# schmidtjonathan/Climate2Weather

Measured on AMD Instinct MI355X. Metric: UNet denoise steps/sec (train fwd+bwd+allreduce+AdamW+EMA windows/s), higher is better.
Workload: dtype bf16; 1 GPU; configs/sda_unet.yml default net, 5 vars x window 13 = 65 ch, 128x128, bf16 training step, 128 windows/GPU/step; global_batch=128, parallelism=dp1, params=72132929

## Files before the change

climate2weather_amd/csrc/conv_igemm.hip:

```cpp
#include <cstdlib>

#include "conv_epilogue.h"
#include "knobs.h"
#include "launch.h"

namespace {

constexpr int BN = 128;
constexpr int WBYTES = BN * 128;
constexpr int NSLOT = 3;
template <int NW> struct GCfg {
    static constexpr int BM = 64 * NW;
    static constexpr int NTHREADS = 128 * NW;
    static constexpr int PBYTES = BM * 128;
    static constexpr int ROWS_PER_ROUND = NTHREADS / 8;
    static constexpr int WROUNDS = BN / ROWS_PER_ROUND;
    static constexpr int ROUND_BYTES = NTHREADS * 16;
};

template <typename T> struct Mma;
template <> struct Mma<bf16_t> {
    __device__ static __forceinline__ void run(const u32x4_t& a, const u32x4_t& b, f32x4_t& c) { c = mfma16<bf16_t>(a, b, c); }
};
template <> struct Mma<f16_t> {
    __device__ static __forceinline__ void run(const u32x4_t& a, const u32x4_t& b, f32x4_t& c) { c = mfma16<f16_t>(a, b, c); }
};
template <> struct Mma<float> {
    __device__ static __forceinline__ void run(const u32x4_t& a, const u32x4_t& b, f32x4_t& c) {
#pragma unroll
        for (int s = 0; s < 4; ++s)
            c = __builtin_amdgcn_mfma_f32_16x16x4f32(__uint_as_float(a[s]), __uint_as_float(b[s]), c, 0, 0, 0);
    }
};

template <typename T, int MODE, int NW>
__global__ __launch_bounds__(GCfg<NW>::NTHREADS, 2) void conv_igemm_kernel(const C2wConvArgs p) {
    constexpr int BM = GCfg<NW>::BM, NTHREADS = GCfg<NW>::NTHREADS, PBYTES = GCfg<NW>::PBYTES;
    constexpr int RPR = GCfg<NW>::ROWS_PER_ROUND, WROUNDS = GCfg<NW>::WROUNDS, RB = GCfg<NW>::ROUND_BYTES;
    constexpr int ESZ = sizeof(T);
    constexpr int NT = (MODE == C2W_CONV_1X1) ? 1 : 9;
    constexpr int CK = 128 / ESZ;
    extern __shared__ __attribute__((aligned(16))) char smem[];
    char* const Pbuf = smem;
    char* const Wbuf = smem + NSLOT * PBYTES;

    const int tid = threadIdx.x;
    const int lane = tid & 63;
    const int wid = __builtin_amdgcn_readfirstlane(tid >> 6);
    const int li = lane & 15, lg = lane >> 4;
    const int wm = wid & 1, wn = wid >> 1;

    const int nN = (p.Cout + BN - 1) / BN;
    const int nblk = gridDim.x;
    int L;
    {
        const int bid = blockIdx.x, xcd = bid & 7, q = nblk >> 3, r = nblk & 7;
        L = (xcd < r ? xcd * (q + 1) : r * (q + 1) + (xcd - r) * q) + (bid >> 3);
    }
    const int tn = L % nN, tm = L / nN;
    const int co0 = tn * BN;
    const int HWo = p.Hout * p.Wout;
    const int npix = p.B * HWo;

    bool par = false;
    int pa = 0, pw = 0, psh = 0;
    const int Wh = p.Wout >> 1, HWq = HWo >> 2, nq = npix >> 2;
    if constexpr (MODE == C2W_CONV_TS2) {
        par = ((p.Hout | p.Wout) & 1) == 0 && nq % BM == 0;
        if (par) {
            const int cls = (tm * BM) / nq;
            pa = cls < 2;
            pw = (cls & 1) == 0;
            psh = pa + pw;
        }
    }
    const int b0 = (MODE == C2W_CONV_TS2 && par) ? ((tm * BM) % nq) / HWq : (tm * BM) / HWo;
    const size_t img_bytes = (size_t)p.Hin * p.Win * p.Cin * ESZ;
    size_t xrem = (size_t)(p.B - b0) * img_bytes;
    if (xrem > 0x7fffffffu) xrem = 0x7fffffffu;
    const __amdgpu_buffer_rsrc_t rx = make_rsrc((const char*)p.x + (size_t)b0 * img_bytes, (uint32_t)xrem);
    const __amdgpu_buffer_rsrc_t rw = make_rsrc(p.w, (uint32_t)((size_t)p.wrows * NT * p.Cin * ESZ));

    auto row_pixel = [&](int Q, int& b, int& oh, int& ow) {
        if (MODE == C2W_CONV_TS2 && par) {
            const int qq = Q % nq;
            b = qq / HWq;
            const int rem = qq - b * HWq;
            const int yh = rem / Wh;
            oh = 2 * yh + pa;
            ow = 2 * (rem - yh * Wh) + pw;
        } else {
            b = Q / HWo;
            const int rem = Q - b * HWo;
            oh = rem / p.Wout;
            ow = rem - oh * p.Wout;
        }
    };

    int pb[4], pyx[4];
    uint32_t plc[4];
#pragma unroll
    for (int i = 0; i < 4; ++i) {
        const int q = (tid >> 3) + RPR * i;
        const int Q = tm * BM + q;
        int b, oh, ow;
        row_pixel(Q, b, oh, ow);
        pb[i] = (Q < npix) ? (b - b0) * p.Hin : -1;
        pyx[i] = (oh << 16) | ow;
        plc[i] = (uint32_t)(((tid & 7) ^ (q & 7)) << 4);
    }
    uint32_t wvo[WROUNDS];
#pragma unroll
    for (int i = 0; i < WROUNDS; ++i) {
        const int row = (tid >> 3) + RPR * i;
        wvo[i] = (uint32_t)(co0 + row) * (uint32_t)(NT * p.Cin * ESZ) + (uint32_t)(((tid & 7) ^ (row & 7)) << 4);
    }

    const int nchunk = p.Cin / CK;
    const int NS = (MODE == C2W_CONV_TS2 && par) ? (nchunk << psh) : nchunk * NT;

    auto issue = [&](int s, int buf) {
        int chunk, kh, kw;
        if (MODE == C2W_CONV_TS2 && par) {
            chunk = s >> psh;
            const int ti = s - (chunk << psh);
            kh = pa ? 2 * (ti >> pw) : 1;
            kw = pw ? 2 * (ti & 1) : 1;
        } else {
            chunk = s / NT;
            const int tap0 = s - chunk * NT;
            kh = tap0 / 3;
            kw = tap0 - kh * 3;
        }
        const int tap = kh * 3 + kw;
        char* const pdst = Pbuf + buf * PBYTES + wid * 1024;
#pragma unroll
        for (int i = 0; i < 4; ++i) {
            int ih, iw;
            const bool ok = src_pixel<MODE>(p, pyx[i] >> 16, pyx[i] & 0xffff, kh, kw, ih, iw) && pb[i] >= 0;
            const uint32_t voff = ok ? (uint32_t)(((pb[i] + ih) * p.Win + iw) * p.Cin) * ESZ + plc[i] : C2W_OOB;
            glds16(rx, pdst + i * RB, voff, (uint32_t)chunk * 128u);
        }
        char* const wdst = Wbuf + buf * WBYTES + wid * 1024;
        const uint32_t wso = (uint32_t)(tap * p.Cin + chunk * CK) * ESZ;
#pragma unroll
        for (int i = 0; i < WROUNDS; ++i) glds16(rw, wdst + i * RB, wvo[i], wso);
    };

    uint32_t offA[4], offB[4];
#pragma unroll
    for (int m = 0; m < 4; ++m) {
        const int row = wm * 64 + m * 16 + li;
        offA[m] = (uint32_t)(row * 128 + ((lg ^ (row & 7)) << 4));
    }
#pragma unroll
    for (int n = 0; n < 4; ++n) {
        const int row = wn * 64 + n * 16 + li;
        offB[n] = (uint32_t)(row * 128 + ((lg ^ (row & 7)) << 4));
    }

    f32x4_t acc[4][4];
#pragma unroll
    for (int m = 0; m < 4; ++m)
#pragma unroll
        for (int n = 0; n < 4; ++n) acc[m][n] = (f32x4_t){0.f, 0.f, 0.f, 0.f};

    float bv[4][4];
    epi_load_bias(p, co0 + wm * 64 + lg * 4, bv);
    issue(0, 0);
    if (NS > 1) issue(1, 1);
    int slot = 0;
    for (int s = 0; s < NS; ++s) {
        if (s + 1 < NS) {
            if constexpr (WROUNDS == 2) {
                asm volatile("s_waitcnt vmcnt(6)" ::: "memory");
            } else {
                asm volatile("s_waitcnt vmcnt(8)" ::: "memory");
            }
        } else {
            asm volatile("s_waitcnt vmcnt(0)" ::: "memory");
        }
        asm volatile("s_waitcnt lgkmcnt(0)" ::: "memory");
        __builtin_amdgcn_s_barrier();
        if (s + 2 < NS) issue(s + 2, slot >= 1 ? slot - 1 : NSLOT - 1);
        const char* const Pb = Pbuf + slot * PBYTES;
        const char* const Wb = Wbuf + slot * WBYTES;
#pragma unroll
        for (int ks = 0; ks < 2; ++ks) {
            u32x4_t a[4], b[4];
#pragma unroll
            for (int m = 0; m < 4; ++m) a[m] = *(const u32x4_t*)(Wb + (offA[m] ^ (ks * 64)));
#pragma unroll
            for (int n = 0; n < 4; ++n) b[n] = *(const u32x4_t*)(Pb + (offB[n] ^ (ks * 64)));
#pragma unroll
            for (int m = 0; m < 4; ++m)
#pragma unroll
                for (int n = 0; n < 4; ++n) Mma<T>::run(a[m], b[n], acc[m][n]);
        }
        slot = slot + 1 == NSLOT ? 0 : slot + 1;
    }

    constexpr int OS = BN * ESZ + 16;
    EpiStore<T, BM, NTHREADS> est;
    est.prefetch(p, tid, co0, [&](int row) -> long long {
        const int Q = tm * BM + row;
        if (Q >= npix) return -1;
        if (MODE == C2W_CONV_TS2 && par) {
            int b, oh, ow;
            row_pixel(Q, b, oh, ow);
            return ((long long)b * p.Hout + oh) * p.Wout + ow;
        }
        return (long long)Q;
    });
    __syncthreads();
    char* const O = smem;
    epi_acc_to_lds<T>(O, OS, acc, bv, p.act, wm * 64, wn * 64, li, lg);
    __syncthreads();
    est.finish(p, O, OS, tid);
}

template <typename T, int MODE>
__global__ void conv_naive_kernel(const C2wConvArgs p) {
    constexpr int NT = (MODE == C2W_CONV_1X1) ? 1 : 9;
    const int HWo = p.Hout * p.Wout;
    const long long total = (long long)p.B * HWo * p.Cout;
    for (long long idx = (long long)blockIdx.x * blockDim.x + threadIdx.x; idx < total; idx += (long long)gridDim.x * blockDim.x) {
        const int co = (int)(idx % p.Cout);
        const long long Q = idx / p.Cout;
        const int b = (int)(Q / HWo);
        const int rem = (int)(Q - (long long)b * HWo);
        const int oh = rem / p.Wout, ow = rem - oh * p.Wout;
        float acc = 0.f;
        for (int tap = 0; tap < NT; ++tap) {
            int ih, iw;
            if (!src_pixel<MODE>(p, oh, ow, tap / 3, tap % 3, ih, iw)) continue;
            const T* xp = (const T*)p.x + (((size_t)b * p.Hin + ih) * p.Win + iw) * p.Cin;
            const T* wp = (const T*)p.w + ((size_t)co * NT + tap) * p.Cin;
            if (co >= p.wrows) continue;
            for (int ci = 0; ci < p.Cin; ++ci) acc = fmaf(Elem<T>::ld(wp + ci), Elem<T>::ld(xp + ci), acc);
        }
        if (p.bias && co < p.wrows) acc += p.bias[co];
        if (p.act == C2W_ACT_SILU) acc = silu_f(acc);
        if (p.act == C2W_ACT_RELU) acc = relu_f(acc);
        const size_t off = (size_t)Q * p.ldy + co;
        if (p.mul) {
            float g = Elem<T>::ld((const T*)p.mul + off);
            acc *= (p.mulmode == C2W_MUL_DSILU) ? dsilu_f(g) : g;
        }
        if (p.res) acc += Elem<T>::ld((const T*)p.res + off);
        if (p.act == C2W_ACT_SILU_PAIR && p.y2) {
            Elem<T>::st((T*)p.y + off, acc);
            const float a_ = Elem<T>::ld((const T*)p.y + off);
            Elem<T>::st((T*)p.y + off, silu_f(a_));
            Elem<T>::st((T*)p.y2 + off, dsilu_f(a_));
            continue;
        }
        if (p.act == C2W_ACT_RELU_PAIR && p.y2) {
            Elem<T>::st((T*)p.y + off, acc);
            const float a_ = Elem<T>::ld((const T*)p.y + off);
            Elem<T>::st((T*)p.y + off, relu_f(a_));
            Elem<T>::st((T*)p.y2 + off, a_ > 0.f ? 1.f : 0.f);
            continue;
        }
        Elem<T>::st((T*)p.y + off, acc);
        if (p.y2) Elem<T>::st((T*)p.y2 + off, silu_f(Elem<T>::ld((const T*)p.y + off)));
    }
}

template <typename T, int MODE, int NW>
int launch_tile(const C2wConvArgs& a, long long npix, int nN, hipStream_t st) {
    typedef GCfg<NW> CF;
    constexpr int ESZ = sizeof(T);
    constexpr int lds_loop = NSLOT * (CF::PBYTES + WBYTES), lds_epi = CF::BM * (BN * ESZ + 16);
    constexpr int lds = lds_loop > lds_epi ? lds_loop : lds_epi;
    if (int rc = c2w_lds_optin<conv_igemm_kernel<T, MODE, NW>>(lds)) return rc;
    const int nM = (int)((npix + CF::BM - 1) / CF::BM);
    conv_igemm_kernel<T, MODE, NW><<<nM * nN, CF::NTHREADS, lds, st>>>(a);
    return (int)hipGetLastError();
}

template <typename T, int MODE>
int launch_mode(const C2wConvArgs& a, int naive, hipStream_t st) {
    const long long npix = (long long)a.B * a.Hout * a.Wout;
    if (naive) {
        long long total = npix * a.Cout;
        int grid = (int)((total + 255) / 256 < 65536 ? (total + 255) / 256 : 65536);
        conv_naive_kernel<T, MODE><<<grid, 256, 0, st>>>(a);
        return (int)hipGetLastError();
    }
    const int nN = (a.Cout + BN - 1) / BN;
    const bool small = ((npix + 255) / 256) * nN < c2w_cu_count();
    return small ? launch_tile<T, MODE, 2>(a, npix, nN, st) : launch_tile<T, MODE, 4>(a, npix, nN, st);
}

template <typename T>
int launch_dtype(const C2wConvArgs& a, int naive, hipStream_t st) {
    switch (a.mode) {
        case C2W_CONV_1X1: return launch_mode<T, C2W_CONV_1X1>(a, naive, st);
        case C2W_CONV_S1: return launch_mode<T, C2W_CONV_S1>(a, naive, st);
        case C2W_CONV_S2: return launch_mode<T, C2W_CONV_S2>(a, naive, st);
        case C2W_CONV_UP: return launch_mode<T, C2W_CONV_UP>(a, naive, st);
        case C2W_CONV_TS2: return launch_mode<T, C2W_CONV_TS2>(a, naive, st);
    }
    return C2W_ERR_BAD_ARG;
}

}

namespace {
C2wKnobs read_knobs() {
    C2wKnobs k;
    k.force_gather = getenv("C2W_FORCE_GATHER") != nullptr;
    k.conv_t3 = getenv("C2W_CONV_T3") ? atoi(getenv("C2W_CONV_T3")) : -1;
    k.conv_s2_patch = getenv("C2W_CONV_S2_PATCH") ? atoi(getenv("C2W_CONV_S2_PATCH")) : 0;
    k.ts2_pairs = !(getenv("C2W_TS2_PAIRS") && atoi(getenv("C2W_TS2_PAIRS")) == 0);
    k.wgrad_atomics = getenv("C2W_WGRAD_ATOMICS") != nullptr;
    k.loss_fusion = getenv("C2W_NO_LOSS_FUSION") == nullptr;
    k.half8 = getenv("C2W_NO_HALF8") == nullptr;
    k.half8_db = !(getenv("C2W_HALF8_DB") && atoi(getenv("C2W_HALF8_DB")) == 0);
    k.attn_valu = getenv("C2W_ATTN_VALU") != nullptr;
    return k;
}
C2wKnobs g_knobs = read_knobs();
}
const C2wKnobs& c2w_knobs() { return g_knobs; }
extern "C" void c2w_knobs_reload(void) { g_knobs = read_knobs(); }

extern "C" int c2w_conv_patch_supported(const C2wConvArgs* a, int dtype) {
    (void)dtype;
    return a != nullptr && c2w_conv_patch_eligible(*a) && !c2w_knobs().force_gather ? 1 : 0;
}

extern "C" int c2w_conv_pool2_supported(const C2wConvArgs* a, int dtype) {
    (void)dtype;
    if (a == nullptr || a->mode != C2W_CONV_S1 || a->res != nullptr || a->mul != nullptr || a->y2 != nullptr || a->act != C2W_ACT_NONE ||
        a->ln_x != nullptr || a->lnf_y != nullptr)
        return 0;
    return c2w_conv_patch_eligible(*a) && !c2w_conv_pair_eligible(*a) && !c2w_knobs().force_gather ? 1 : 0;
}

extern "C" int c2w_conv_lnfwd_supported(const C2wConvArgs* a, int dtype) {
    if (a == nullptr || (dtype != C2W_DTYPE_BF16 && dtype != C2W_DTYPE_F16)) return 0;
    if (a->Cout != 128 || a->ldy != 128 || a->mul != nullptr || a->y2 != nullptr || a->act != C2W_ACT_NONE || a->ln_x != nullptr) return 0;
    return c2w_conv_patch_eligible(*a) && !c2w_knobs().force_gather ? 1 : 0;
}

extern "C" int c2w_conv_lnbwd_supported(const C2wConvArgs* a, int dtype) {
    if (a == nullptr || (dtype != C2W_DTYPE_BF16 && dtype != C2W_DTYPE_F16)) return 0;
    if (a->Cout != 128 || a->ldy != 128 || a->mul != nullptr || a->y2 != nullptr || a->act != C2W_ACT_NONE) return 0;
    return c2w_conv_patch_eligible(*a) && !c2w_knobs().force_gather ? 1 : 0;
}

int c2w_conv_splitk_plan_impl(const C2wConvArgs& a, int dtype, unsigned long long* ws_bytes);
extern "C" int c2w_conv_splitk_plan(const C2wConvArgs* a, int dtype, unsigned long long* ws_bytes) {
    if (a == nullptr) return C2W_ERR_BAD_ARG;
    return c2w_conv_splitk_plan_impl(*a, dtype, ws_bytes);
}

extern "C" int c2w_conv_lnfwd_chain_supported(const C2wConvArgs* a, int dtype) {
    if (!c2w_conv_lnfwd_supported(a, dtype)) return 0;
    return a->mode == C2W_CONV_S1 && c2w_conv_patch3_wanted(*a, dtype) ? 1 : 0;
}

extern "C" int c2w_conv_loss_supported(const C2wConvArgs* a, int dtype) {
    if (a == nullptr || (dtype != C2W_DTYPE_BF16 && dtype != C2W_DTYPE_F16)) return 0;
    if (a->mode != C2W_CONV_S1 || a->wrows > 80 || a->Cout > 128 || a->ldy != 128 || a->res != nullptr || a->mul != nullptr || a->y2 != nullptr ||
        a->act != C2W_ACT_NONE || a->ln_x != nullptr || a->lnf_y != nullptr || (a->flags & C2W_CONV_POOL2) != 0)
        return 0;
    if (a->loss_sum != nullptr && (a->loss_eps == nullptr || a->loss_C <= 0 || a->loss_C != a->wrows || (a->loss_lde & 7) != 0 || a->loss_lde < a->loss_C ||
                                   a->loss_lde > 128))
        return 0;
    const C2wKnobs& k = c2w_knobs();
    return !k.force_gather && k.loss_fusion && c2w_conv_patch_eligible(*a) && c2w_conv_patch3_wanted(*a, dtype) ? 1 : 0;
}

extern "C" long long c2w_conv_det_scratch_bytes(const C2wConvArgs* a, int dtype) {
    if (a == nullptr) return C2W_ERR_BAD_ARG;
    if (a->ln_x != nullptr && a->ln_dm != nullptr) {
        if (!c2w_conv_lnbwd_supported(a, dtype)) return C2W_ERR_UNSUPPORTED;
        return (long long)a->B * (a->Hout >> 3) * (a->Wout >> 4) * 128 * (long long)sizeof(float);
    }
    if (a->loss_sum != nullptr) {
        C2wConvArgs g = *a;
        g.loss_sum = nullptr;
        if (!c2w_conv_loss_supported(&g, dtype)) return C2W_ERR_UNSUPPORTED;
        return (long long)a->B * (a->Hout >> 4) * (a->Wout >> 4) * ((a->Cout + 127) / 128) * (long long)sizeof(float);
    }
    return 0;
}

extern "C" int c2w_conv_wpacked_supported(const C2wConvArgs* a, int dtype) {
    if (a == nullptr || (dtype != C2W_DTYPE_BF16 && dtype != C2W_DTYPE_F16)) return 0;
    return !c2w_knobs().force_gather && c2w_conv_patch_eligible(*a) && c2w_conv_patch3_wanted(*a, dtype) ? 1 : 0;
}

extern "C" int c2w_conv_dispatch(const C2wConvArgs* a, int dtype) {
    if (a == nullptr) return C2W_ERR_BAD_ARG;
    const bool gather = c2w_knobs().force_gather;
    if (!gather && c2w_conv_patch_eligible(*a)) return c2w_conv_patch3_wanted(*a, dtype) ? C2W_KERNEL_PATCH_16X16 : C2W_KERNEL_PATCH_8X16;
    if (!gather && c2w_conv_pair_eligible(*a)) return C2W_KERNEL_PATCH_PAIR;
    if (!gather && c2w_conv_ts2_patch_eligible(*a)) return C2W_KERNEL_PATCH_TS2;
    if (!gather && c2w_conv_s2_patch_eligible(*a, dtype)) return C2W_KERNEL_PATCH_S2;
    return C2W_KERNEL_GATHER;
}

extern "C" int c2w_conv_forward(const C2wConvArgs* a, int dtype, int naive, void* stream) {
    if (a == nullptr || a->x == nullptr || a->w == nullptr || a->y == nullptr) return C2W_ERR_BAD_ARG;
    const int esz = dtype == C2W_DTYPE_F32 ? 4 : 2;
    const int ck = 128 / esz;
    if (a->Cin <= 0 || a->Cin % ck != 0) return C2W_ERR_BAD_SHAPE;
    if (a->Cout <= 0 || a->Cout % (16 / esz) != 0 || a->ldy % (16 / esz) != 0) return C2W_ERR_BAD_SHAPE;
    if (a->B <= 0 || a->Hin <= 0 || a->Win <= 0 || a->Hout <= 0 || a->Wout <= 0) return C2W_ERR_BAD_SHAPE;
    if (a->Hout >= 65536 || a->Wout >= 65536) return C2W_ERR_BAD_SHAPE;
    if (a->act < C2W_ACT_NONE || a->act > C2W_ACT_RELU_PAIR) return C2W_ERR_BAD_ARG;
    if ((a->act == C2W_ACT_SILU_PAIR || a->act == C2W_ACT_RELU_PAIR) && a->y2 == nullptr) return C2W_ERR_BAD_ARG;
    hipStream_t st = (hipStream_t)stream;
    if (a->ln_x != nullptr && (naive != 0 || !c2w_conv_lnbwd_supported(a, dtype))) return C2W_ERR_BAD_SHAPE;
    if (a->lnf_y != nullptr && (naive != 0 || !c2w_conv_lnfwd_supported(a, dtype))) return C2W_ERR_BAD_SHAPE;
    if ((a->ln_rstd != nullptr && a->ln_x == nullptr) || (a->lnf_rstd != nullptr && a->lnf_y == nullptr)) return C2W_ERR_BAD_ARG;
    if (a->lnf_mean != nullptr || a->res_rstd != nullptr || a->res_mean != nullptr || a->res_m != nullptr || (a->flags & C2W_CONV_NO_Y) != 0) {
        if (a->lnf_y == nullptr || (a->res_rstd == nullptr) != (a->res_mean == nullptr) || (a->res_m != nullptr && a->res_rstd == nullptr) ||
            (a->res_rstd != nullptr && a->res == nullptr))
            return C2W_ERR_BAD_ARG;
        if (naive != 0 || !c2w_conv_lnfwd_chain_supported(a, dtype)) return C2W_ERR_BAD_SHAPE;
    }
    if ((a->flags & C2W_CONV_POOL2) != 0 && (naive != 0 || !c2w_conv_pool2_supported(a, dtype))) return C2W_ERR_BAD_SHAPE;
    if (a->loss_sum != nullptr && (naive != 0 || !c2w_conv_loss_supported(a, dtype))) return C2W_ERR_BAD_SHAPE;
    if ((a->flags & C2W_CONV_DETERMINISTIC) != 0 && ((a->ln_x != nullptr && a->ln_dm != nullptr) || a->loss_sum != nullptr)) {
        const long long need = c2w_conv_det_scratch_bytes(a, dtype);
        if (need < 0 || a->det_ws == nullptr || a->det_ws_bytes < (unsigned long long)need) return C2W_ERR_BAD_ARG;
    }
    if (a->splitk > 1) {
        unsigned long long need = 0;
        if (naive != 0 || a->splitk_ws == nullptr || c2w_conv_splitk_plan_impl(*a, dtype, &need) != a->splitk || a->splitk_ws_bytes < need) return C2W_ERR_BAD_SHAPE;
    }
    if ((a->flags & C2W_CONV_WPACKED) != 0 && (naive != 0 || !c2w_conv_wpacked_supported(a, dtype))) return C2W_ERR_BAD_SHAPE;
    const bool patch = naive == 0 && !c2w_knobs().force_gather;
    if (patch && c2w_conv_patch_eligible(*a)) return c2w_conv_patch_s1(*a, dtype, st);
    if (patch && c2w_conv_pair_eligible(*a)) return c2w_conv_patch_pair(*a, dtype, st);
    if (patch && c2w_conv_ts2_patch_eligible(*a)) return c2w_conv_patch_ts2(*a, dtype, st);
    if (patch && c2w_conv_s2_patch_eligible(*a, dtype)) return c2w_conv_patch_s2(*a, dtype, st);
    if (naive == 2) naive = 0;
    return c2w_by_dtype(dtype, [&](auto t) { return launch_dtype<decltype(t)>(*a, naive, st); });
}
```

climate2weather_amd/csrc/knobs.h:

```cpp
#pragma once

struct C2wKnobs {
    bool force_gather;
    int conv_t3;
    int conv_s2_patch;
    bool ts2_pairs;
    bool wgrad_atomics;
    bool attn_valu;
    bool loss_fusion;
    bool half8;
    bool half8_db;
};

const C2wKnobs& c2w_knobs();
extern "C" void c2w_knobs_reload(void);
```

climate2weather_amd/csrc/wgrad.hip:

```cpp
#include <cstdint>
#include <cstdlib>

#include "conv_geom.h"
#include "knobs.h"
#include "launch.h"

namespace {

constexpr int KT = 64;
constexpr int NTHREADS = 512;
constexpr int ABYTES = KT * 256;
constexpr int BBYTES = KT * 512;
constexpr int NSLOT = 3;

struct WgradArgs {
    const void* dy;
    const void* x;
    float* dw;
    float* db;
    int B, Hin, Win, Cin, Hout, Wout, Cout, ldy;
    int nsplit, ktiles_per_split;
    FastDiv div_hw, div_w;
    float* ws;
    float* wsb;
    int det;
};

__device__ __forceinline__ uint32_t swz(int row) { return (uint32_t)(((row & 3) << 2) | ((row >> 2) & 3)); }

struct WgItem {
    const void* dy;
    const void* x;
    float* dw;
    float* db;
};
constexpr int WG_MAX_ITEMS = 16;
struct WgradGroupArgs {
    WgradArgs c;
    int n, live_per_item;
    unsigned long long ws_item_floats;
    unsigned long long wsb_item_floats;
    WgItem item[WG_MAX_ITEMS];
};

__device__ __forceinline__ int wg_xcd_order(int bid, int nblk) {
    const int xcd = bid & 7, q = nblk >> 3, r = nblk & 7;
    return (xcd < r ? xcd * (q + 1) : r * (q + 1) + (xcd - r) * q) + (bid >> 3);
}

template <typename T, int MODE>
__device__ __forceinline__ void wgrad_body(const WgradArgs& p, const int L) {
    constexpr int ESZ = sizeof(T);
    constexpr int NT = (MODE == C2W_CONV_1X1) ? 1 : 9;
    constexpr int COT = 256 / ESZ;
    constexpr int CIB = 128 / ESZ;
    constexpr int MT = (ESZ == 2) ? 4 : 2;
    constexpr int NTL = MT;
    extern __shared__ __attribute__((aligned(16))) char smem[];
    char* const Abuf = smem;
    char* const Bbuf = smem + NSLOT * ABYTES;

    const int tid = threadIdx.x, lane = tid & 63;
    const int wid = __builtin_amdgcn_readfirstlane(tid >> 6);
    const int li = lane & 15, lg = lane >> 4;
    const int wm = wid & 1, wn = wid >> 1;

    const int cib_per_tap = p.Cin / CIB;
    const int nb_total = NT * cib_per_tap;
    const int tilesN = (nb_total + 3) / 4;
    const int tilesM = (p.Cout + COT - 1) / COT;
    const int tilesMN = tilesM * tilesN;
    const int split = L / tilesMN, mn = L - split * tilesMN;
    const int tm = mn / tilesN, tn = mn - tm * tilesN;
    const int co0 = tm * COT;
    const int HWo = p.Hout * p.Wout;
    const int npix = p.B * HWo;
    const int nkt = (npix + KT - 1) / KT;
    const int kt0 = split * p.ktiles_per_split;
    const int kt1 = (kt0 + p.ktiles_per_split < nkt) ? kt0 + p.ktiles_per_split : nkt;

    uint32_t avo[2];
#pragma unroll
    for (int i = 0; i < 2; ++i) {
        const int s = tid + NTHREADS * i, row = s >> 4, pc = s & 15;
        const uint32_t lc = (uint32_t)pc ^ swz(row);
        const int c = co0 + (int)lc * (16 / ESZ);
        avo[i] = (c < p.Cout) ? (uint32_t)row * (uint32_t)(p.ldy * ESZ) + (uint32_t)c * ESZ : C2W_OOB;
    }
    int brow[4], btap[4];
    uint32_t bco[4];
#pragma unroll
    for (int i = 0; i < 4; ++i) {
        const int s = tid + NTHREADS * i, row = s >> 5, pc = s & 31;
        const uint32_t lc = (uint32_t)pc ^ swz(row);
        const int nb = tn * 4 + (int)(lc >> 3);
        const int tap = nb / cib_per_tap;
        brow[i] = row;
        btap[i] = (nb < nb_total) ? tap : -1;
        bco[i] = (uint32_t)((nb - tap * cib_per_tap) * 128 + (lc & 7) * 16);
    }
    const size_t img_bytes = (size_t)p.Hin * p.Win * p.Cin * ESZ;
    const size_t dy_total = (size_t)npix * p.ldy * ESZ;

    auto issue = [&](int kt, int buf) {
        const int q0 = kt * KT;
        const size_t aoff = (size_t)q0 * p.ldy * ESZ;
        size_t arem = dy_total - aoff;
        if (arem > 0x7fffffffu) arem = 0x7fffffffu;
        const __amdgpu_buffer_rsrc_t ra = make_rsrc((const char*)p.dy + aoff, (uint32_t)arem);
        char* const adst = Abuf + buf * ABYTES + wid * 1024;
#pragma unroll
        for (int i = 0; i < 2; ++i) glds16(ra, adst + i * 8192, avo[i], 0);
        const int b0 = fast_div(q0, p.div_hw);
        size_t xrem = (size_t)(p.B - b0) * img_bytes;
        if (xrem > 0x7fffffffu) xrem = 0x7fffffffu;
        const __amdgpu_buffer_rsrc_t rx = make_rsrc((const char*)p.x + (size_t)b0 * img_bytes, (uint32_t)xrem);
        char* const bdst = Bbuf + buf * BBYTES + wid * 1024;
#pragma unroll
        for (int i = 0; i < 4; ++i) {
            const int Q = q0 + brow[i];
            const int b = fast_div(Q, p.div_hw);
            const int rem = Q - b * HWo;
            const int oh = fast_div(rem, p.div_w);
            const int ow = rem - oh * p.Wout;
            const int tap = btap[i];
            const int kh = tap / 3, kw = tap - kh * 3;
            int ih, iw;
            const bool ok = src_pixel<MODE>(p, oh, ow, kh, kw, ih, iw) && tap >= 0 && Q < npix;
            const uint32_t voff = ok ? (uint32_t)((((b - b0) * p.Hin + ih) * p.Win + iw) * p.Cin) * ESZ + bco[i] : C2W_OOB;
            glds16(rx, bdst + i * 8192, voff, 0);
        }
    };

    f32x4_t acc[MT][NTL];
#pragma unroll
    for (int m = 0; m < MT; ++m)
#pragma unroll
        for (int n = 0; n < NTL; ++n) acc[m][n] = (f32x4_t){0.f, 0.f, 0.f, 0.f};

    const bool do_bias = p.db != nullptr && tn == 0 && wn == 0;
    f32x4_t accb[MT];
#pragma unroll
    for (int m = 0; m < MT; ++m) accb[m] = (f32x4_t){0.f, 0.f, 0.f, 0.f};

    uint32_t offA[MT][2], offB[NTL][2];
    if constexpr (ESZ == 2) {
        const int q = li >> 2, pp = li & 3;
#pragma unroll
        for (int h = 0; h < 2; ++h) {
            const int row = 8 * lg + q + 4 * h;
            const uint32_t f = swz(row);
#pragma unroll
            for (int m = 0; m < MT; ++m)
                offA[m][h] = (uint32_t)(row * 256 + ((((wm * 8 + m * 2 + (pp >> 1)) ^ f) & 15) << 4) + 8 * (pp & 1));
#pragma unroll
            for (int n = 0; n < NTL; ++n) {
                const uint32_t lcg = (uint32_t)(wn * 8 + n * 2 + (pp >> 1));
                offB[n][h] = (uint32_t)(row * 512 + ((lcg ^ f) << 4) + 8 * (pp & 1));
            }
        }
    } else {
#pragma unroll
        for (int m = 0; m < MT; ++m) {
            offA[m][0] = (uint32_t)((wm * 8 + m * 4 + (li >> 2)) ^ (lg << 2));
            offA[m][1] = (uint32_t)((li & 3) * 4);
        }
#pragma unroll
        for (int n = 0; n < NTL; ++n) {
            offB[n][0] = (uint32_t)((wn * 8 + n * 4 + (li >> 2)) ^ (lg << 2));
            offB[n][1] = (uint32_t)((li & 3) * 4);
        }
    }

    if (kt0 < kt1) issue(kt0, 0);
    if (kt0 + 1 < kt1) issue(kt0 + 1, 1);
    int buf = 0;
    for (int kt = kt0; kt < kt1; ++kt) {
        if (kt + 1 < kt1) {
            asm volatile("s_waitcnt vmcnt(6)" ::: "memory");
        } else {
            asm volatile("s_waitcnt vmcnt(0)" ::: "memory");
        }
        __builtin_amdgcn_s_barrier();
        if (kt + 2 < kt1) issue(kt + 2, buf >= 1 ? buf - 1 : NSLOT - 1);
        const char* const Ab = Abuf + buf * ABYTES;
        const char* const Bb = Bbuf + buf * BBYTES;
        if constexpr (ESZ == 2) {
            const uint32_t sA = (uint32_t)(uintptr_t)Ab, sB = (uint32_t)(uintptr_t)Bb;
            auto rd = [&](tr_frag& f, uint32_t base, uint32_t o0, uint32_t o1, auto IMMc) {
                constexpr int IMM = decltype(IMMc)::value;
                asm volatile("ds_read_b64_tr_b16 %0, %1 offset:%2" : "=v"(f.lo) : "v"(base + o0), "n"(IMM));
                asm volatile("ds_read_b64_tr_b16 %0, %1 offset:%2" : "=v"(f.hi) : "v"(base + o1), "n"(IMM));
            };
            static_for<2>([&](auto KSc) {
                constexpr int ks = decltype(KSc)::value;
                tr_frag a[MT], b[NTL];
#pragma unroll
                for (int m = 0; m < MT; ++m) rd(a[m], sA, offA[m][0], offA[m][1], IC<ks * 32 * 256>{});
                rd(b[0], sB, offB[0][0], offB[0][1], IC<ks * 32 * 512>{});
                rd(b[1], sB, offB[1][0], offB[1][1], IC<ks * 32 * 512>{});
                static_for<NTL>([&](auto Nc) {
                    constexpr int n = decltype(Nc)::value;
                    if constexpr (n + 2 < NTL) rd(b[n + 2], sB, offB[n + 2][0], offB[n + 2][1], IC<ks * 32 * 512>{});
                    constexpr int AHEAD = 2 * ((n + 2 < NTL ? n + 2 : NTL - 1) - n);
                    if constexpr (AHEAD == 4) asm volatile("s_waitcnt lgkmcnt(4)" ::: "memory");
                    else if constexpr (AHEAD == 2) asm volatile("s_waitcnt lgkmcnt(2)" ::: "memory");
                    else asm volatile("s_waitcnt lgkmcnt(0)" ::: "memory");
                    __builtin_amdgcn_sched_barrier(0);
                    const bf16x8_t bv = b[n].vec();
#pragma unroll
                    for (int m = 0; m < MT; ++m) acc[m][n] = mfma16s<T>(a[m].vec(), bv, acc[m][n]);
                    if (n == NTL - 1 && do_bias) {
                        const bf16x8_t ones = __builtin_bit_cast(bf16x8_t, ones16<T>());
#pragma unroll
                        for (int m = 0; m < MT; ++m) accb[m] = mfma16s<T>(a[m].vec(), ones, accb[m]);
                    }
                    __builtin_amdgcn_sched_barrier(0);
                });
            });
        } else {
#pragma unroll
            for (int kk = 0; kk < 16; ++kk) {
                const int row = kk * 4 + lg;
                float a[MT], b[NTL];
#pragma unroll
                for (int m = 0; m < MT; ++m) a[m] = *(const float*)(Ab + row * 256 + ((offA[m][0] ^ (kk & 3)) << 4) + offA[m][1]);
#pragma unroll
                for (int n = 0; n < NTL; ++n) b[n] = *(const float*)(Bb + row * 512 + ((offB[n][0] ^ (kk & 3)) << 4) + offB[n][1]);
#pragma unroll
                for (int m = 0; m < MT; ++m)
#pragma unroll
                    for (int n = 0; n < NTL; ++n) acc[m][n] = __builtin_amdgcn_mfma_f32_16x16x4f32(a[m], b[n], acc[m][n], 0, 0, 0);
                if (do_bias) {
#pragma unroll
                    for (int m = 0; m < MT; ++m) accb[m] = __builtin_amdgcn_mfma_f32_16x16x4f32(a[m], 1.0f, accb[m], 0, 0, 0);
                }
            }
        }
        buf = buf + 1 == NSLOT ? 0 : buf + 1;
    }

    constexpr int NCOL = 4 * CIB;
    constexpr int OS = NCOL + 4;
    __syncthreads();
    float* const O = (float*)smem;
#pragma unroll
    for (int m = 0; m < MT; ++m)
#pragma unroll
        for (int n = 0; n < NTL; ++n) {
            const int col = wn * CIB + n * 16 + li;
#pragma unroll
            for (int r = 0; r < 4; ++r) O[(wm * (COT / 2) + m * 16 + lg * 4 + r) * OS + col] = acc[m][n][r];
        }
    __syncthreads();
    if (kt0 >= kt1) return;
    if (do_bias && li == 0) {
#pragma unroll
        for (int m = 0; m < MT; ++m)
#pragma unroll
            for (int r = 0; r < 4; ++r) {
                const int row = wm * (COT / 2) + m * 16 + lg * 4 + r;
                const int co = co0 + row;
                if (p.det) {
                    if (p.wsb != nullptr) p.wsb[((size_t)split * tilesM + tm) * COT + row] = accb[m][r];
                    else if (co < p.Cout) p.db[co] = p.db[co] + accb[m][r];
                } else if (co < p.Cout) {
                    atomicAdd(p.db + co, accb[m][r]);
                }
            }
    }
    if (p.ws != nullptr) {
        float* const dst = p.ws + ((size_t)split * tilesMN + mn) * (COT * NCOL);
        for (int idx = tid; idx < COT * NCOL; idx += NTHREADS) dst[idx] = O[(idx / NCOL) * OS + (idx % NCOL)];
        return;
    }
    for (int idx = tid; idx < COT * NCOL; idx += NTHREADS) {
        const int row = idx / NCOL, col = idx - row * NCOL;
        const int cb = col / CIB, cil = col - cb * CIB;
        const int nb = tn * 4 + cb;
        const int co = co0 + row;
        if (nb < nb_total && co < p.Cout) {
            const int tap = nb / cib_per_tap;
            const int ci = (nb - tap * cib_per_tap) * CIB + cil;
            atomicAdd(p.dw + ((size_t)co * NT + tap) * p.Cin + ci, O[row * OS + col]);
        }
    }
}

template <typename T, int MODE>
__global__ __launch_bounds__(NTHREADS, 2) void wgrad_kernel(const WgradArgs p) {
    wgrad_body<T, MODE>(p, wg_xcd_order((int)blockIdx.x, (int)gridDim.x));
}

__device__ __forceinline__ WgItem wg_item(int it) {
    typedef __attribute__((address_space(4))) const char karg_t;
    const WgItem __attribute__((address_space(4)))* tab =
        (const WgItem __attribute__((address_space(4)))*)((karg_t*)__builtin_amdgcn_kernarg_segment_ptr() + offsetof(WgradGroupArgs, item));
    WgItem r;
    r.dy = tab[it].dy;
    r.x = tab[it].x;
    r.dw = tab[it].dw;
    r.db = tab[it].db;
    return r;
}

template <typename T, int MODE>
__global__ __launch_bounds__(NTHREADS, 2) void wgrad_group_kernel(const WgradGroupArgs g) {
    const int Lg = wg_xcd_order((int)blockIdx.x, (int)gridDim.x);
    const int it = __builtin_amdgcn_readfirstlane(Lg / g.live_per_item);
    const WgItem e = wg_item(it);
    WgradArgs p = g.c;
    p.dy = e.dy;
    p.x = e.x;
    p.dw = e.dw;
    p.db = e.db;
    p.ws = g.c.ws != nullptr ? g.c.ws + (size_t)it * g.ws_item_floats : nullptr;
    p.wsb = g.c.wsb != nullptr ? g.c.wsb + (size_t)it * g.wsb_item_floats : nullptr;
    wgrad_body<T, MODE>(p, Lg - it * g.live_per_item);
}

struct WgradBiasReduce {
    const float* wsb;
    float* db;
    int cols, tpo, nmain;
};
static inline WgradBiasReduce bias_reduce_of(const float* wsb, float* db, int cols, int nsplit, int nmain) {
    WgradBiasReduce br;
    br.wsb = wsb; br.db = db; br.cols = cols; br.tpo = det_reduce_tpo(nsplit); br.nmain = nmain;
    return br;
}

template <int COT, int CIB, int NT>
__device__ __forceinline__ void wgrad_gather_reduce_body(const float* __restrict__ ws, float* __restrict__ dw, int nsplit, int tilesM,
                                                         int tilesN, int Cin, int Cout, int nblk) {
    constexpr int NCOL = 4 * CIB;
    __shared__ f32x4_t red[4][64];
    const size_t per4 = (size_t)tilesM * tilesN * COT * NCOL / 4;
    const f32x4_t* ws4 = (const f32x4_t*)ws;
    const int q = threadIdx.x & 63, grp = threadIdx.x >> 6;
    const int cib_per_tap = Cin / CIB, nb_total = NT * cib_per_tap;
    for (size_t base = (size_t)blockIdx.x * 64; base < per4; base += (size_t)nblk * 64) {
        const size_t i4 = base + q;
        f32x4_t acc = {0.f, 0.f, 0.f, 0.f};
        if (i4 < per4) {
#pragma unroll 8
            for (int sidx = grp; sidx < nsplit; sidx += 4) acc += ws4[(size_t)sidx * per4 + i4];
        }
        red[grp][q] = acc;
        __syncthreads();
        if (grp == 0 && i4 < per4) {
            acc = red[0][q] + red[1][q] + red[2][q] + red[3][q];
            const size_t i = i4 * 4;
            const int col = (int)(i % NCOL);
            size_t r = i / NCOL;
            const int row = (int)(r % COT);
            const int mn = (int)(r / COT);
            const int tm = mn / tilesN, tn = mn - tm * tilesN;
            const int cb = col / CIB, cil = col - cb * CIB;
            const int nb = tn * 4 + cb;
            const int co = tm * COT + row;
            if (nb < nb_total && co < Cout) {
                const int tap = nb / cib_per_tap;
                const int ci = (nb - tap * cib_per_tap) * CIB + cil;
                f32x4_t* d = (f32x4_t*)(dw + ((size_t)co * NT + tap) * Cin + ci);
                *d = *d + acc;
            }
        }
        __syncthreads();
    }
}

template <int COT, int CIB, int NT>
__global__ __launch_bounds__(256) void wgrad_gather_reduce_kernel(const float* __restrict__ ws, float* __restrict__ dw, int nsplit, int tilesM,
                                                                  int tilesN, int Cin, int Cout, WgradBiasReduce br) {
    if ((int)blockIdx.x >= br.nmain) {
        det_reduce_body(br.wsb, br.db, nsplit, Cout, Cout, 0, br.tpo, br.cols, (int)blockIdx.x - br.nmain);
        return;
    }
    wgrad_gather_reduce_body<COT, CIB, NT>(ws, dw, nsplit, tilesM, tilesN, Cin, Cout, br.nmain);
}
template <int COT, int CIB, int NT>
__global__ __launch_bounds__(256) void wgrad_gather_reduce_group_kernel(const WgradGroupArgs g, int nsplit, int tilesM, int tilesN, WgradBiasReduce br) {
    const int it = (int)blockIdx.y;
    const WgItem e = wg_item(it);
    if ((int)blockIdx.x >= br.nmain) {
        if (e.db != nullptr)
            det_reduce_body(g.c.wsb + (size_t)it * g.wsb_item_floats, e.db, nsplit, g.c.Cout, g.c.Cout, 0, br.tpo, br.cols, (int)blockIdx.x - br.nmain);
        return;
    }
    wgrad_gather_reduce_body<COT, CIB, NT>(g.c.ws + (size_t)it * g.ws_item_floats, e.dw, nsplit, tilesM, tilesN, g.c.Cin, g.c.Cout, br.nmain);
}

FastDiv make_div(uint32_t d) {
    FastDiv r{0, 0};
    if (d <= 1) return r;
    uint32_t s = 0;
    while ((1ull << s) < d) ++s;
    r.magic = (uint32_t)(((1ull << (31 + s)) + d - 1) / d);
    r.shift = s - 1;
    return r;
}

template <int ESZ, int NT>
static void split_plan(const C2wConvArgs& a, int& tilesM, int& tilesN, int& nsplit, int& ktiles_per_split) {
    constexpr int COT = 256 / ESZ, CIB = 128 / ESZ;
    const long long npix = (long long)a.B * a.Hout * a.Wout;
    const int nkt = (int)((npix + KT - 1) / KT);
    tilesN = (NT * (a.Cin / CIB) + 3) / 4;
    tilesM = (a.Cout + COT - 1) / COT;
    const int tilesMN = tilesM * tilesN;
    constexpr int target = 432;
    nsplit = (target + tilesMN - 1) / tilesMN;
    if (nsplit > nkt) nsplit = nkt;
    if (nsplit < 1) nsplit = 1;
    ktiles_per_split = (nkt + nsplit - 1) / nsplit;
    nsplit = (nkt + ktiles_per_split - 1) / ktiles_per_split;
}

template <int ESZ, int NT>
static size_t ws_need(const C2wConvArgs& a) {
    constexpr int COT = 256 / ESZ, CIB = 128 / ESZ;
    int tilesM, tilesN, nsplit, per;
    split_plan<ESZ, NT>(a, tilesM, tilesN, nsplit, per);
    const size_t bias_rows = (a.flags & C2W_CONV_DETERMINISTIC) ? (size_t)nsplit * tilesM * COT * sizeof(float) : 0;
    return nsplit > 1 ? (size_t)nsplit * tilesM * tilesN * COT * 4 * CIB * sizeof(float) + bias_rows : 0;
}

template <typename T, int MODE>
int launch(const C2wConvArgs& a, float* dw, float* db, float* ws, size_t ws_bytes, hipStream_t st) {
    constexpr int ESZ = sizeof(T);
    constexpr int NT = (MODE == C2W_CONV_1X1) ? 1 : 9;
    constexpr int COT = 256 / ESZ, CIB = 128 / ESZ;
    WgradArgs p;
    p.dy = a.y; p.x = a.x; p.dw = dw; p.db = db;
    p.B = a.B; p.Hin = a.Hin; p.Win = a.Win; p.Cin = a.Cin; p.Hout = a.Hout; p.Wout = a.Wout; p.Cout = a.Cout; p.ldy = a.ldy;
    int tilesM, tilesN;
    split_plan<ESZ, NT>(a, tilesM, tilesN, p.nsplit, p.ktiles_per_split);
    const int tilesMN = tilesM * tilesN;
    p.div_hw = make_div((uint32_t)(a.Hout * a.Wout));
    p.div_w = make_div((uint32_t)a.Wout);
    constexpr int lds_main = NSLOT * (ABYTES + BBYTES);
    constexpr int lds_epi = COT * (4 * CIB + 4) * 4;
    constexpr int lds = lds_main > lds_epi ? lds_main : lds_epi;
    if (int rc = c2w_lds_optin<wgrad_kernel<T, MODE>>(lds)) return rc;
    const size_t need = (size_t)p.nsplit * tilesMN * COT * 4 * CIB * sizeof(float);
    p.det = (a.flags & C2W_CONV_DETERMINISTIC) ? 1 : 0;
    if (p.det) {
        if (c2w_knobs().wgrad_atomics) return C2W_ERR_BAD_ARG;
        if (p.nsplit > 1 && (ws == nullptr || need + (size_t)p.nsplit * tilesM * COT * sizeof(float) > ws_bytes)) return C2W_ERR_BAD_ARG;
    }
    p.ws = (ws != nullptr && need <= ws_bytes && p.nsplit > 1 && !c2w_knobs().wgrad_atomics) ? ws : nullptr;
    p.wsb = p.det && p.nsplit > 1 && db != nullptr ? ws + need / sizeof(float) : nullptr;
    wgrad_kernel<T, MODE><<<tilesMN * p.nsplit, NTHREADS, lds, st>>>(p);
    if (p.ws != nullptr) {
        const size_t per4 = (size_t)tilesMN * COT * 4 * CIB / 4;
        const int grid = (int)((per4 + 63) / 64 < 4096 ? (per4 + 63) / 64 : 4096);
        const int extra = p.wsb != nullptr ? det_reduce_blocks(p.nsplit, a.Cout) : 0;
        wgrad_gather_reduce_kernel<COT, CIB, NT><<<grid + extra, 256, 0, st>>>(p.ws, dw, p.nsplit, tilesM, tilesN, a.Cin, a.Cout,
                                                                               bias_reduce_of(p.wsb, db, tilesM * COT, p.nsplit, grid));
    }
    return (int)hipGetLastError();
}

template <typename T>
int launch_dtype(const C2wConvArgs& a, float* dw, float* db, float* ws, size_t ws_bytes, hipStream_t st) {
    switch (a.mode) {
        case C2W_CONV_1X1: return launch<T, C2W_CONV_1X1>(a, dw, db, ws, ws_bytes, st);
        case C2W_CONV_S1: return launch<T, C2W_CONV_S1>(a, dw, db, ws, ws_bytes, st);
        case C2W_CONV_S2: return launch<T, C2W_CONV_S2>(a, dw, db, ws, ws_bytes, st);
        case C2W_CONV_UP: return launch<T, C2W_CONV_UP>(a, dw, db, ws, ws_bytes, st);
    }
    return C2W_ERR_BAD_ARG;
}

static void gather_group_plan(int n, int tilesMN, int nkt, int& nsplit, int& per) {
    nsplit = 480 / (n * tilesMN);
    if (nsplit > nkt) nsplit = nkt;
    if (nsplit < 1) nsplit = 1;
    per = (nkt + nsplit - 1) / nsplit;
    nsplit = (nkt + per - 1) / per;
}

template <int ESZ, int NT>
static size_t gather_group_ws_need(const C2wConvArgs& a, int n) {
    constexpr int COT = 256 / ESZ, CIB = 128 / ESZ;
    int tilesM, tilesN, ns1, per1, nsplit, per;
    split_plan<ESZ, NT>(a, tilesM, tilesN, ns1, per1);
    const long long npix = (long long)a.B * a.Hout * a.Wout;
    gather_group_plan(n, tilesM * tilesN, (int)((npix + KT - 1) / KT), nsplit, per);
    const size_t bias_rows = (a.flags & C2W_CONV_DETERMINISTIC) ? (size_t)n * nsplit * tilesM * COT * sizeof(float) : 0;
    return nsplit > 1 ? (size_t)n * nsplit * tilesM * tilesN * COT * 4 * CIB * sizeof(float) + bias_rows : 0;
}

template <typename T, int MODE>
int launch_group(const C2wConvArgs& a, const C2wWgradItem* items, int n, float* ws, size_t ws_bytes, hipStream_t st) {
    constexpr int ESZ = sizeof(T);
    constexpr int NT = (MODE == C2W_CONV_1X1) ? 1 : 9;
    constexpr int COT = 256 / ESZ, CIB = 128 / ESZ;
    WgradGroupArgs g;
    WgradArgs& p = g.c;
    p.dy = nullptr; p.x = nullptr; p.dw = nullptr; p.db = nullptr;
    p.B = a.B; p.Hin = a.Hin; p.Win = a.Win; p.Cin = a.Cin; p.Hout = a.Hout; p.Wout = a.Wout; p.Cout = a.Cout; p.ldy = a.ldy;
    int tilesM, tilesN, ns1, per1;
    split_plan<ESZ, NT>(a, tilesM, tilesN, ns1, per1);
    const int tilesMN = tilesM * tilesN;
    const long long npix = (long long)a.B * a.Hout * a.Wout;
    gather_group_plan(n, tilesMN, (int)((npix + KT - 1) / KT), p.nsplit, p.ktiles_per_split);
    p.div_hw = make_div((uint32_t)(a.Hout * a.Wout));
    p.div_w = make_div((uint32_t)a.Wout);
    const size_t item_floats = (size_t)p.nsplit * tilesMN * COT * 4 * CIB;
    p.det = (a.flags & C2W_CONV_DETERMINISTIC) ? 1 : 0;
    const size_t bias_item_floats = p.det ? (size_t)p.nsplit * tilesM * COT : 0;
    if (p.nsplit > 1 && (ws == nullptr || (size_t)n * (item_floats + bias_item_floats) * sizeof(float) > ws_bytes)) return C2W_ERR_BAD_ARG;
    p.wsb = p.det && p.nsplit > 1 ? ws + (size_t)n * item_floats : nullptr;
    g.wsb_item_floats = bias_item_floats;
    p.ws = p.nsplit > 1 ? ws : nullptr;
    g.n = n;
    g.live_per_item = tilesMN * p.nsplit;
    g.ws_item_floats = item_floats;
    for (int i = 0; i < WG_MAX_ITEMS; ++i) {
        const C2wWgradItem& e = items[i < n ? i : n - 1];
        g.item[i].dy = e.dy; g.item[i].x = e.x; g.item[i].dw = e.dw; g.item[i].db = e.dbias;
    }
    constexpr int lds_main = NSLOT * (ABYTES + BBYTES);
    constexpr int lds_epi = COT * (4 * CIB + 4) * 4;
    constexpr int lds = lds_main > lds_epi ? lds_main : lds_epi;
    if (int rc = c2w_lds_optin<wgrad_group_kernel<T, MODE>>(lds)) return rc;
    wgrad_group_kernel<T, MODE><<<g.live_per_item * n, NTHREADS, lds, st>>>(g);
    if (p.ws != nullptr) {
        const size_t per4 = (size_t)tilesMN * COT * 4 * CIB / 4;
        const int grid = (int)((per4 + 63) / 64 < 4096 ? (per4 + 63) / 64 : 4096);
        const int extra = p.wsb != nullptr ? det_reduce_blocks(p.nsplit, a.Cout) : 0;
        wgrad_gather_reduce_group_kernel<COT, CIB, NT><<<dim3(grid + extra, n), 256, 0, st>>>(g, p.nsplit, tilesM, tilesN,
                                                                                              bias_reduce_of(p.wsb, nullptr, tilesM * COT, p.nsplit, grid));
    }
    return (int)hipGetLastError();
}

}

static int wgrad_check(const C2wConvArgs* a, int dtype) {
    if (a == nullptr) return C2W_ERR_BAD_ARG;
    if (dtype != C2W_DTYPE_F32 && dtype != C2W_DTYPE_BF16 && dtype != C2W_DTYPE_F16) return C2W_ERR_BAD_ARG;
    const int esz = dtype == C2W_DTYPE_F32 ? 4 : 2;
    if (a->Cin <= 0 || a->Cin % (128 / esz) != 0) return C2W_ERR_BAD_SHAPE;
    if (a->Cout <= 0 || a->ldy % (16 / esz) != 0 || a->Cout > a->ldy) return C2W_ERR_BAD_SHAPE;
    if (a->B <= 0 || a->Hin <= 0 || a->Win <= 0 || a->Hout <= 0 || a->Wout <= 0) return C2W_ERR_BAD_SHAPE;
    if ((long long)a->B * a->Hout * a->Wout >= (1ll << 31)) return C2W_ERR_BAD_SHAPE;
    if (a->mode != C2W_CONV_1X1 && a->mode != C2W_CONV_S1 && a->mode != C2W_CONV_S2 && a->mode != C2W_CONV_UP) return C2W_ERR_BAD_ARG;
    return 0;
}

extern "C" int c2w_conv_wgrad(const C2wConvArgs* a, float* dw, float* dbias, void* workspace, unsigned long long workspace_bytes, int dtype,
                              void* stream) {
    const int rc = wgrad_check(a, dtype);
    if (rc != 0) return rc;
    if (a->x == nullptr || a->y == nullptr || dw == nullptr) return C2W_ERR_BAD_ARG;
    hipStream_t st = (hipStream_t)stream;
    float* ws = (float*)workspace;
    const size_t wsb = workspace == nullptr ? 0 : (size_t)workspace_bytes;
    if (c2w_wgrad_patch_eligible(*a) && !c2w_knobs().force_gather) return c2w_wgrad_patch(*a, dw, dbias, ws, wsb, dtype, st);
    return c2w_by_dtype(dtype, [&](auto t) { return launch_dtype<decltype(t)>(*a, dw, dbias, ws, wsb, st); });
}

static bool gather_group_eligible(const C2wConvArgs& a, int n) {
    return a.mode == C2W_CONV_1X1 && n >= 2 && n <= WG_MAX_ITEMS && !c2w_knobs().wgrad_atomics;
}

extern "C" int c2w_conv_wgrad_grouped_supported(const C2wConvArgs* a, int n, int dtype) {
    if (wgrad_check(a, dtype) != 0) return 0;
    if (c2w_wgrad_patch_group_eligible(*a, n, dtype) && !c2w_knobs().force_gather) return 1;
    return gather_group_eligible(*a, n) ? 1 : 0;
}

extern "C" long long c2w_conv_wgrad_grouped_workspace_bytes(const C2wConvArgs* a, int n, int dtype) {
    const int rc = wgrad_check(a, dtype);
    if (rc != 0) return rc;
    if (!c2w_conv_wgrad_grouped_supported(a, n, dtype)) return C2W_ERR_UNSUPPORTED;
    if (c2w_wgrad_patch_group_eligible(*a, n, dtype) && !c2w_knobs().force_gather) return (long long)c2w_wgrad_patch_group_ws_bytes(*a, n, dtype);
    return (long long)(dtype == C2W_DTYPE_F32 ? gather_group_ws_need<4, 1>(*a, n) : gather_group_ws_need<2, 1>(*a, n));
}

extern "C" int c2w_conv_wgrad_grouped(const C2wConvArgs* a, const C2wWgradItem* items, int n, void* workspace, unsigned long long workspace_bytes,
                                      int dtype, void* stream) {
    const int rc = wgrad_check(a, dtype);
    if (rc != 0) return rc;
    if (items == nullptr || n < 1) return C2W_ERR_BAD_ARG;
    for (int i = 0; i < n; ++i)
        if (items[i].x == nullptr || items[i].dy == nullptr || items[i].dw == nullptr) return C2W_ERR_BAD_ARG;
    if (!c2w_conv_wgrad_grouped_supported(a, n, dtype)) return C2W_ERR_UNSUPPORTED;
    float* const ws = (float*)workspace;
    const size_t wsb = workspace == nullptr ? 0 : (size_t)workspace_bytes;
    hipStream_t st = (hipStream_t)stream;
    if (c2w_wgrad_patch_group_eligible(*a, n, dtype) && !c2w_knobs().force_gather) return c2w_wgrad_patch_group(*a, items, n, ws, wsb, dtype, st);
    return c2w_by_dtype(dtype, [&](auto t) { return launch_group<decltype(t), C2W_CONV_1X1>(*a, items, n, ws, wsb, st); });
}

extern "C" int c2w_conv_wgrad_dispatch(const C2wConvArgs* a, int dtype) {
    const int rc = wgrad_check(a, dtype);
    if (rc != 0) return rc;
    if (c2w_wgrad_patch_eligible(*a) && !c2w_knobs().force_gather) return c2w_wgrad_patch_pair(*a) ? C2W_KERNEL_PATCH_PAIR : C2W_KERNEL_PATCH_8X16;
    return C2W_KERNEL_GATHER;
}

extern "C" long long c2w_conv_wgrad_workspace_bytes(const C2wConvArgs* a, int dtype) {
    const int rc = wgrad_check(a, dtype);
    if (rc != 0) return rc;
    if (c2w_wgrad_patch_eligible(*a) && !c2w_knobs().force_gather) return (long long)c2w_wgrad_patch_ws_bytes(*a, dtype);
    const int esz = dtype == C2W_DTYPE_F32 ? 4 : 2;
    if (a->mode == C2W_CONV_1X1) return (long long)(esz == 4 ? ws_need<4, 1>(*a) : ws_need<2, 1>(*a));
    return (long long)(esz == 4 ? ws_need<4, 9>(*a) : ws_need<2, 9>(*a));
}
```

Before: 2778 windows/s.

## Use two-slot LDS ring for bf16 1x1 conv and retune 1x1 wgrad split

Templates the conv implicit-GEMM kernel on ring depth and generalises the vmcnt waits and prologue to it. For 16-bit 1x1 convs with enough tiles, it launches a 2-warp tile with a 2-slot ring so two workgroups fit per CU's LDS. The gain in occupancy costs prefetch depth. Separately, the grouped 1x1 weight-gradient split count is now sized from the CU count (one or two waves) instead of a fixed 480. This may add workspace or reduction cost.

```diff
diff --git a/climate2weather_amd/csrc/conv_igemm.hip b/climate2weather_amd/csrc/conv_igemm.hip
--- a/climate2weather_amd/csrc/conv_igemm.hip
+++ b/climate2weather_amd/csrc/conv_igemm.hip
@@ -9,6 +9,8 @@
 constexpr int BN = 128;
 constexpr int WBYTES = BN * 128;
 constexpr int NSLOT = 3;
+constexpr int NSLOT_1X1 = 2;
+constexpr int CU_LDS_BYTES = 160 * 1024;
 template <int NW> struct GCfg {
     static constexpr int BM = 64 * NW;
     static constexpr int NTHREADS = 128 * NW;
@@ -33,7 +35,23 @@
     }
 };
 
-template <typename T, int MODE, int NW>
+template <int N> __device__ __forceinline__ void wait_vmcnt() {
+    static_assert(N >= 0 && N < 64, "vmcnt is a 6-bit field");
+    asm volatile("s_waitcnt vmcnt(%0)" ::"n"(N) : "memory");
+}
+template <int LPS, int K> __device__ __forceinline__ void wait_stage_landed(int s, int NS) {
+    if constexpr (K == 0) {
+        wait_vmcnt<0>();
+    } else {
+        if (s + K < NS) {
+            wait_vmcnt<K * LPS>();
+        } else {
+            wait_stage_landed<LPS, K - 1>(s, NS);
+        }
+    }
+}
+
+template <typename T, int MODE, int NW, int D>
 __global__ __launch_bounds__(GCfg<NW>::NTHREADS, 2) void conv_igemm_kernel(const C2wConvArgs p) {
     constexpr int BM = GCfg<NW>::BM, NTHREADS = GCfg<NW>::NTHREADS, PBYTES = GCfg<NW>::PBYTES;
     constexpr int RPR = GCfg<NW>::ROWS_PER_ROUND, WROUNDS = GCfg<NW>::WROUNDS, RB = GCfg<NW>::ROUND_BYTES;
@@ -41,8 +59,10 @@
     constexpr int NT = (MODE == C2W_CONV_1X1) ? 1 : 9;
     constexpr int CK = 128 / ESZ;
     extern __shared__ __attribute__((aligned(16))) char smem[];
+    constexpr int AHEAD = D - 1;
+    constexpr int LPS = 4 + WROUNDS;
     char* const Pbuf = smem;
-    char* const Wbuf = smem + NSLOT * PBYTES;
+    char* const Wbuf = smem + D * PBYTES;
 
     const int tid = threadIdx.x;
     const int lane = tid & 63;
@@ -168,21 +188,22 @@
     float bv[4][4];
     epi_load_bias(p, co0 + wm * 64 + lg * 4, bv);
     issue(0, 0);
-    if (NS > 1) issue(1, 1);
+    static_assert(AHEAD >= 1 && AHEAD <= 4, "prologue written out for rings of 2 to 5 slots");
+    if constexpr (AHEAD > 1) {
+        if (NS > 1) issue(1, 1);
+    }
+    if constexpr (AHEAD > 2) {
+        if (NS > 2) issue(2, 2);
+    }
+    if constexpr (AHEAD > 3) {
+        if (NS > 3) issue(3, 3);
+    }
     int slot = 0;
     for (int s = 0; s < NS; ++s) {
-        if (s + 1 < NS) {
-            if constexpr (WROUNDS == 2) {
-                asm volatile("s_waitcnt vmcnt(6)" ::: "memory");
-            } else {
-                asm volatile("s_waitcnt vmcnt(8)" ::: "memory");
-            }
-        } else {
-            asm volatile("s_waitcnt vmcnt(0)" ::: "memory");
-        }
+        wait_stage_landed<LPS, AHEAD - 1>(s, NS);
         asm volatile("s_waitcnt lgkmcnt(0)" ::: "memory");
         __builtin_amdgcn_s_barrier();
-        if (s + 2 < NS) issue(s + 2, slot >= 1 ? slot - 1 : NSLOT - 1);
+        if (s + AHEAD < NS) issue(s + AHEAD, slot >= 1 ? slot - 1 : D - 1);
         const char* const Pb = Pbuf + slot * PBYTES;
         const char* const Wb = Wbuf + slot * WBYTES;
 #pragma unroll
@@ -197,7 +218,7 @@
 #pragma unroll
                 for (int n = 0; n < 4; ++n) Mma<T>::run(a[m], b[n], acc[m][n]);
         }
-        slot = slot + 1 == NSLOT ? 0 : slot + 1;
+        slot = slot + 1 == D ? 0 : slot + 1;
     }
 
     constexpr int OS = BN * ESZ + 16;
@@ -267,15 +288,16 @@
     }
 }
 
-template <typename T, int MODE, int NW>
+template <typename T, int MODE, int NW, int D = NSLOT>
 int launch_tile(const C2wConvArgs& a, long long npix, int nN, hipStream_t st) {
     typedef GCfg<NW> CF;
     constexpr int ESZ = sizeof(T);
-    constexpr int lds_loop = NSLOT * (CF::PBYTES + WBYTES), lds_epi = CF::BM * (BN * ESZ + 16);
+    constexpr int lds_loop = D * (CF::PBYTES + WBYTES), lds_epi = CF::BM * (BN * ESZ + 16);
     constexpr int lds = lds_loop > lds_epi ? lds_loop : lds_epi;
-    if (int rc = c2w_lds_optin<conv_igemm_kernel<T, MODE, NW>>(lds)) return rc;
+    static_assert(lds <= CU_LDS_BYTES, "the ring does not fit a CU");
+    if (int rc = c2w_lds_optin<conv_igemm_kernel<T, MODE, NW, D>>(lds)) return rc;
     const int nM = (int)((npix + CF::BM - 1) / CF::BM);
-    conv_igemm_kernel<T, MODE, NW><<<nM * nN, CF::NTHREADS, lds, st>>>(a);
+    conv_igemm_kernel<T, MODE, NW, D><<<nM * nN, CF::NTHREADS, lds, st>>>(a);
     return (int)hipGetLastError();
 }
 
@@ -289,6 +311,10 @@
         return (int)hipGetLastError();
     }
     const int nN = (a.Cout + BN - 1) / BN;
+    if constexpr (MODE == C2W_CONV_1X1 && sizeof(T) == 2) {
+        static_assert(CU_LDS_BYTES / (NSLOT_1X1 * (GCfg<2>::PBYTES + WBYTES)) == 2, "the 1x1 ring is planned at two workgroups per CU");
+        if (c2w_knobs().conv_1x1_ring && ((npix + 127) / 128) * nN > c2w_cu_count()) return launch_tile<T, MODE, 2, NSLOT_1X1>(a, npix, nN, st);
+    }
     const bool small = ((npix + 255) / 256) * nN < c2w_cu_count();
     return small ? launch_tile<T, MODE, 2>(a, npix, nN, st) : launch_tile<T, MODE, 4>(a, npix, nN, st);
 }
@@ -319,6 +345,7 @@
     k.half8 = getenv("C2W_NO_HALF8") == nullptr;
     k.half8_db = !(getenv("C2W_HALF8_DB") && atoi(getenv("C2W_HALF8_DB")) == 0);
     k.attn_valu = getenv("C2W_ATTN_VALU") != nullptr;
+    k.conv_1x1_ring = !(getenv("C2W_CONV_1X1_RING") && atoi(getenv("C2W_CONV_1X1_RING")) == 0);
     return k;
 }
 C2wKnobs g_knobs = read_knobs();
diff --git a/climate2weather_amd/csrc/knobs.h b/climate2weather_amd/csrc/knobs.h
--- a/climate2weather_amd/csrc/knobs.h
+++ b/climate2weather_amd/csrc/knobs.h
@@ -9,6 +9,7 @@
     bool attn_valu;
     bool loss_fusion;
     bool half8;
+    bool conv_1x1_ring;
     bool half8_db;
 };
 
diff --git a/climate2weather_amd/csrc/wgrad.hip b/climate2weather_amd/csrc/wgrad.hip
--- a/climate2weather_amd/csrc/wgrad.hip
+++ b/climate2weather_amd/csrc/wgrad.hip
@@ -473,8 +473,14 @@
     return C2W_ERR_BAD_ARG;
 }
 
-static void gather_group_plan(int n, int tilesMN, int nkt, int& nsplit, int& per) {
-    nsplit = 480 / (n * tilesMN);
+static void gather_group_plan(int n, int tilesMN, int nkt, bool one_tap, int& nsplit, int& per) {
+    const int tiles = n * tilesMN;
+    nsplit = 480 / tiles;
+    if (one_tap) {
+        const int cus = c2w_cu_count();
+        nsplit = cus / tiles;
+        if (nsplit * tiles * 5 < cus * 4) nsplit = 2 * cus / tiles;
+    }
     if (nsplit > nkt) nsplit = nkt;
     if (nsplit < 1) nsplit = 1;
     per = (nkt + nsplit - 1) / nsplit;
@@ -487,7 +493,7 @@
     int tilesM, tilesN, ns1, per1, nsplit, per;
     split_plan<ESZ, NT>(a, tilesM, tilesN, ns1, per1);
     const long long npix = (long long)a.B * a.Hout * a.Wout;
-    gather_group_plan(n, tilesM * tilesN, (int)((npix + KT - 1) / KT), nsplit, per);
+    gather_group_plan(n, tilesM * tilesN, (int)((npix + KT - 1) / KT), NT == 1, nsplit, per);
     const size_t bias_rows = (a.flags & C2W_CONV_DETERMINISTIC) ? (size_t)n * nsplit * tilesM * COT * sizeof(float) : 0;
     return nsplit > 1 ? (size_t)n * nsplit * tilesM * tilesN * COT * 4 * CIB * sizeof(float) + bias_rows : 0;
 }
@@ -505,7 +511,7 @@
     split_plan<ESZ, NT>(a, tilesM, tilesN, ns1, per1);
     const int tilesMN = tilesM * tilesN;
     const long long npix = (long long)a.B * a.Hout * a.Wout;
-    gather_group_plan(n, tilesMN, (int)((npix + KT - 1) / KT), p.nsplit, p.ktiles_per_split);
+    gather_group_plan(n, tilesMN, (int)((npix + KT - 1) / KT), NT == 1, p.nsplit, p.ktiles_per_split);
     p.div_hw = make_div((uint32_t)(a.Hout * a.Wout));
     p.div_w = make_div((uint32_t)a.Wout);
     const size_t item_floats = (size_t)p.nsplit * tilesMN * COT * 4 * CIB;
```

New measurement: 2778 windows/s (median of 2 runs). About the same (-0.0%).
